# microsoft/AI2BMD

Hardware: NVIDIA H100
Metric: MD steps/sec (higher is better)
Workload: dtype f32

## Files before the change

ai2bmd_b200/csrc/engine.cu:

```cuda
#include <cuda_runtime.h>
#include <cxxabi.h>

#include <algorithm>
#include <cmath>
#include <cstdarg>
#include <cstdio>
#include <cstdlib>
#include <cstring>
#include <mutex>
#include <string>
#include <vector>

#include "../../include/visnet_b200.h"
#include "k_edge.cuh"
#include "k_caph.cuh"
#include "k_comm.cuh"
#include "k_edge_tc.cuh"
#include "k_graph_embed.cuh"
#include <nvtx3/nvToolsExt.h>
#include "k_head.cuh"
#include "k_md.cuh"
#include "k_nonbonded.cuh"
#include "k_node.cuh"
#include "k_node2.cuh"
// ... 383 lines not shown
    const int blocks = std::max(1, std::min(tiles, h->sm_count * occ));
    Lc.launch(edge_fwd_kernel<TE, NW>, dim3(blocks), dim3(NW * 32), edge_fwd_smem_bytes<TE>(), a);
    Lc.check();
}
template <int TE, int NW>
void launch_edge_bwd(Launcher& Lc, int l, int occ) {
    vb_handle* h = Lc.h;
    EdgeArgs a{l, h->mw, h->ws};
    const int tiles = (h->ws.Ecap + TE - 1) / TE;
    const int blocks = std::max(1, std::min(tiles, h->sm_count * occ));
    Lc.launch(edge_bwd_kernel<TE, NW>, dim3(blocks), dim3(NW * 32), edge_bwd_smem_bytes<TE>(), a);
    Lc.check();
}

template <int NB>
void launch_node_fwd2(Launcher& Lc, int k) {
    vb_handle* h = Lc.h;
    NodeArgs a{k, h->mw, h->ws, h->timeline ? h->d_tl + (size_t)2 * L * TC_TL_SLOTS + (size_t)k * N2_TL_SLOTS : nullptr, h->krot};
    Lc.launch(node_fwd2_kernel<NB>, dim3((h->ws.N + NB - 1) / NB), dim3(N2Cfg<NB>::THREADS), sizeof(NodeFwd2Smem<NB>), a);
    Lc.check();
}
template <int NB>
void launch_node_bwd2(Launcher& Lc, int k) {
    vb_handle* h = Lc.h;
    NodeArgs a{k, h->mw, h->ws, h->timeline ? h->d_tl + (size_t)2 * L * TC_TL_SLOTS + (size_t)(L + 1 + k) * N2_TL_SLOTS : nullptr, h->krot};
    Lc.launch(node_bwd2_kernel<NB>, dim3((h->ws.N + NB - 1) / NB), dim3(N2Cfg<NB>::THREADS), sizeof(NodeBwd2Smem<NB>), a);
    Lc.check();
}
int node_nb(const vb_handle* h) {
    if (h->node_nb > 0) return h->node_nb;
    for (int nb = 1; nb <= 4; nb++)
        if ((h->ws.N + nb - 1) / nb <= h->sm_count) return nb;
    return 8;
}
void node_fwd(Launcher& Lc, int k) {
    if (Lc.h->npw == 2) launch_node_fwd2<16>(Lc, k);
    else switch (node_nb(Lc.h)) {
        case 1: launch_node_fwd2<1>(Lc, k); break;
        case 2: launch_node_fwd2<2>(Lc, k); break;
        case 3: launch_node_fwd2<3>(Lc, k); break;
        case 4: launch_node_fwd2<4>(Lc, k); break;
        default: launch_node_fwd2<8>(Lc, k);
    }
}
void node_bwd(Launcher& Lc, int k) {
    switch (node_nb(Lc.h)) {
        case 1: launch_node_bwd2<1>(Lc, k); break;
        case 2: launch_node_bwd2<2>(Lc, k); break;
        case 3: launch_node_bwd2<3>(Lc, k); break;
        case 4: launch_node_bwd2<4>(Lc, k); break;
        default: launch_node_bwd2<8>(Lc, k);
    }
}
void head(Launcher& Lc) {
    vb_handle* h = Lc.h;
    if (h->ws.N <= 4096) {
        Lc.launch(head2_kernel, dim3(h->ws.N), dim3(128), 0, h->mw, h->ws);
        Lc.check();
        return;
    }
    h->npw == 2 ? launch_head<2>(Lc) : launch_head<1>(Lc);
}
void launch_edge_fwd_tc(Launcher& Lc, int l) {
    vb_handle* h = Lc.h;
    EdgeTcArgs a{};
    a.layer = l; a.mw = h->mw; a.ws = h->ws;
    const LayerW& lw = h->mw.layer[l];
    const size_t chunk = 4 * 8192;
    int n = 0;
    a.jobs[n++] = TcJob{lw.tcW1, 0};
    a.jobs[n++] = TcJob{lw.tcW1 + chunk, 0};
    if (l < L - 1) a.jobs[n++] = TcJob{lw.tcW1 + 2 * chunk, 0};
    a.jobs[n++] = TcJob{lw.tcWs, 0};
    a.jobs[n++] = TcJob{lw.tcWs + chunk, 0};
    a.njobs = n;
    a.tl = h->timeline ? h->d_tl + (size_t)l * TC_TL_SLOTS : nullptr;
    a.tile_rows = h->tile_rows;
    const int rows = h->tc_rows;
    const int tiles = (h->ws.Ecap + h->tile_rows - 1) / h->tile_rows;
    const int blocks = std::max(1, std::min(tiles, h->sm_count));
    if (rows == 32) Lc.launch(edge_fwd_tc_kernel<32>, dim3(blocks), dim3(TC2_THREADS), TC_SMEM_BYTES, a);
    else if (rows == 64) Lc.launch(edge_fwd_tc_kernel<64>, dim3(blocks), dim3(TC2_THREADS), TC_SMEM_BYTES, a);
    else if (rows == 96) Lc.launch(edge_fwd_tc_kernel<96>, dim3(blocks), dim3(TC2_THREADS), TC_SMEM_BYTES, a);
    else Lc.launch(edge_fwd_tc_kernel<128>, dim3(blocks), dim3(TC2_THREADS), TC_SMEM_BYTES, a);
    Lc.check();
}

void edge_fwd(Launcher& Lc, int l) {
    if (Lc.h->edge_tc & 1) { launch_edge_fwd_tc(Lc, l); return; }
    if (Lc.h->te_fwd == 64) launch_edge_fwd<64, 8>(Lc, l, 2);
    else launch_edge_fwd<32, 8>(Lc, l, 4);
}
void launch_edge_bwd_tc(Launcher& Lc, int l) {
    vb_handle* h = Lc.h;
    EdgeTcArgs a{};
    a.layer = l; a.mw = h->mw; a.ws = h->ws;
    const LayerW& lw = h->mw.layer[l];
    const size_t chunk = 4 * 8192;
    const bool upd = l < L - 1;
    int n = 0;
    a.jobs[n++] = TcJob{lw.tcWsN, 0};
    a.jobs[n++] = TcJob{lw.tcWsN + chunk, 1};
    a.jobs[n++] = TcJob{lw.tcW1N + chunk, 0};
    a.jobs[n++] = TcJob{lw.tcW1N, 1};
    if (upd) a.jobs[n++] = TcJob{lw.tcW1N + 2 * chunk, 1};
    a.njobs = n;
    a.tl = h->timeline ? h->d_tl + (size_t)(L + l) * TC_TL_SLOTS : nullptr;
    a.tile_rows = h->tile_rows;
    const int rows = h->tc_rows;
    const int tiles = (h->ws.Ecap + h->tile_rows - 1) / h->tile_rows;
// ... 134 lines not shown
            node_fwd_tc(Lc, l);
            snprintf(name, sizeof(name), "edge_fwd%d", l);
            if (Lc.next(name)) edge_fwd(Lc, l);
        }
        node_fwd_tc(Lc, L);
        if (Lc.next("head")) head(Lc);
        for (int l = L - 1; l >= 0; l--) {
            node_bwd_tc(Lc, l + 1);
            snprintf(name, sizeof(name), "edge_bwd%d", l);
            if (Lc.next(name)) edge_bwd(Lc, l);
        }
        node_bwd_tc(Lc, 0);
    } else {
        for (int l = 0; l < L; l++) {
            snprintf(name, sizeof(name), "node_fwd%d", l);
            if (Lc.next(name)) node_fwd(Lc, l);
            snprintf(name, sizeof(name), "edge_fwd%d", l);
            if (Lc.next(name)) edge_fwd(Lc, l);
        }
        if (Lc.next("node_fwd6")) node_fwd(Lc, L);
        if (Lc.next("head")) head(Lc);
        for (int l = L - 1; l >= 0; l--) {
            snprintf(name, sizeof(name), "node_bwd%d", l + 1);
            if (Lc.next(name)) node_bwd(Lc, l + 1);
            snprintf(name, sizeof(name), "edge_bwd%d", l);
            if (Lc.next(name)) edge_bwd(Lc, l);
        }
        if (Lc.next("node_bwd0")) node_bwd(Lc, 0);
    }
    if (Lc.next("embed_edge_bwd")) {
        const int bb = std::max(1, std::min((ws.Ecap + EEB_WARPS - 1) / EEB_WARPS, h->sm_count * 4));
        Lc.launch(embed_edge_bwd_kernel, dim3(bb), dim3(EEB_WARPS * 32), 0, h->mw, ws);
        Lc.check();
    }
    if (Lc.next("embed_node_bwd")) {
        Lc.launch(embed_node_bwd_kernel, dim3(batch_bwd ? std::min(N, 5 * h->sm_count) : N), dim3(ENB_WARPS * 32), 0, h->mw, ws, io.forces);
        Lc.check();
    }
    if (Lc.next("finalize")) enqueue_finalize(Lc, io);
}

template <typename K>
cudaError_t opt_in_smem(K kernel, size_t bytes) {
    return cudaFuncSetAttribute(kernel, cudaFuncAttributeMaxDynamicSharedMemorySize, (int)bytes);
}

int configure_kernels(vb_handle* h) {
    CUDA_TRY(h, opt_in_smem(edge_fwd_kernel<32, 8>, edge_fwd_smem_bytes<32>()));
    CUDA_TRY(h, opt_in_smem(edge_fwd_kernel<64, 8>, edge_fwd_smem_bytes<64>()));
    CUDA_TRY(h, opt_in_smem(edge_bwd_kernel<32, 8>, edge_bwd_smem_bytes<32>()));
    CUDA_TRY(h, opt_in_smem(edge_bwd_kernel<64, 8>, edge_bwd_smem_bytes<64>()));
    CUDA_TRY(h, opt_in_smem(head_kernel<1>, HeadSmem<1>::BYTES));
    CUDA_TRY(h, opt_in_smem(head_kernel<2>, HeadSmem<2>::BYTES));
    CUDA_TRY(h, opt_in_smem(edge_fwd_tc_kernel<32>, TC_SMEM_BYTES));
    CUDA_TRY(h, opt_in_smem(edge_fwd_tc_kernel<64>, TC_SMEM_BYTES));
    CUDA_TRY(h, opt_in_smem(edge_fwd_tc_kernel<96>, TC_SMEM_BYTES));
    CUDA_TRY(h, opt_in_smem(edge_fwd_tc_kernel<128>, TC_SMEM_BYTES));
    CUDA_TRY(h, opt_in_smem(edge_bwd_tc_kernel<32>, TC_SMEM_BYTES));
    CUDA_TRY(h, opt_in_smem(edge_bwd_tc_kernel<64>, TC_SMEM_BYTES));
    CUDA_TRY(h, opt_in_smem(edge_bwd_tc_kernel<96>, TC_SMEM_BYTES));
    CUDA_TRY(h, opt_in_smem(edge_bwd_tc_kernel<128>, TC_SMEM_BYTES));
    CUDA_TRY(h, opt_in_smem(node_tc_kernel<NT_OPROJ>, TC_SMEM_BYTES));
    CUDA_TRY(h, opt_in_smem(node_tc_kernel<NT_PROJ>, TC_SMEM_BYTES));
    CUDA_TRY(h, opt_in_smem(node_tc_kernel<NT_BWDA>, TC_SMEM_BYTES));
    CUDA_TRY(h, opt_in_smem(node_tc_kernel<NT_BWDB>, TC_SMEM_BYTES));

    CUDA_TRY(h, opt_in_smem(node_fwd2_kernel<1>, sizeof(NodeFwd2Smem<1>)));
    CUDA_TRY(h, opt_in_smem(node_bwd2_kernel<1>, sizeof(NodeBwd2Smem<1>)));
    CUDA_TRY(h, opt_in_smem(node_fwd2_kernel<2>, sizeof(NodeFwd2Smem<2>)));
    CUDA_TRY(h, opt_in_smem(node_bwd2_kernel<2>, sizeof(NodeBwd2Smem<2>)));
    CUDA_TRY(h, opt_in_smem(node_fwd2_kernel<3>, sizeof(NodeFwd2Smem<3>)));
    CUDA_TRY(h, opt_in_smem(node_bwd2_kernel<3>, sizeof(NodeBwd2Smem<3>)));
    CUDA_TRY(h, opt_in_smem(node_fwd2_kernel<4>, sizeof(NodeFwd2Smem<4>)));
    CUDA_TRY(h, opt_in_smem(node_bwd2_kernel<4>, sizeof(NodeBwd2Smem<4>)));
    CUDA_TRY(h, opt_in_smem(node_fwd2_kernel<8>, sizeof(NodeFwd2Smem<8>)));
    CUDA_TRY(h, opt_in_smem(node_fwd2_kernel<16>, sizeof(NodeFwd2Smem<16>)));
    CUDA_TRY(h, opt_in_smem(node_bwd2_kernel<8>, sizeof(NodeBwd2Smem<8>)));
    return VB_OK;
}

int clean_accumulators(vb_handle* h, cudaStream_t st) {
    const Workspace& ws = h->ws;
    const size_t N = ws.N;
    CUDA_TRY(h, cudaMemsetAsync(ws.XA, 0, N * D * 4, st));
    CUDA_TRY(h, cudaMemsetAsync(ws.VA, 0, N * 3 * D * 4, st));
    CUDA_TRY(h, cudaMemsetAsync(ws.GQKV, 0, N * 3 * D * 4, st));
    CUDA_TRY(h, cudaMemsetAsync(ws.GVNMSG, 0, N * 3 * D * 4, st));
    CUDA_TRY(h, cudaMemsetAsync(ws.GTU, 0, N * 6 * D * 4, st));
    CUDA_TRY(h, cudaMemsetAsync(ws.GX, 0, N * D * 4, st));
    CUDA_TRY(h, cudaMemsetAsync(ws.GXA, 0, 3 * N * D * 4, st));
    h->accum_dirty = false;
    return VB_OK;
}

enum { K_EVAL = 0, K_HOST = 1, K_MD_EVAL = 2, K_MD_STEP = 3 };

template <typename F>
int run_cached(vb_handle* h, cudaStream_t st, int kind, const StepIO& io, F&& enqueue) {
    if (h->accum_dirty) { if (int rc = clean_accumulators(h, st)) return rc; }
    if (!h->use_graph) return enqueue(st);
    for (auto& g : h->graphs)
        if (g.kind == kind && g.io == io) { CUDA_TRY(h, cudaGraphLaunch(g.exec, st)); return VB_OK; }
    cudaGraphExec_t exec = nullptr;
    for (int attempt = 0; attempt < 2 && !exec; attempt++) {
        cudaGraph_t graph = nullptr;
        CUDA_TRY(h, cudaStreamBeginCapture(h->own_stream, cudaStreamCaptureModeThreadLocal));
// ... 1206 lines not shown
```

ai2bmd_b200/csrc/k_head.cuh:

```cuda
#pragma once
#include "k_node.cuh"

namespace vb {

template <int NPW>
struct HeadSmem {
    static constexpr int L128 = D + LDS_PAD;
    static constexpr int L256 = 2 * D + LDS_PAD;
    static constexpr int L64 = 64 + LDS_PAD;
    static constexpr int OFF_VS = 0;
    static constexpr int OFF_CAT = OFF_VS + 3 * NPW * L128;
    static constexpr int OFF_HS = OFF_CAT + NPW * L256;
    static constexpr int OFF_YS = OFF_HS + NPW * L128;
    static constexpr int OFF_VP = OFF_YS + NPW * L128;
    static constexpr int OFF_CB = OFF_VP + 3 * NPW * L64;
    static constexpr int OFF_GPB = OFF_CB + NPW * L128;
    static constexpr int OFF_GPRE = OFF_GPB + NPW * L64;
    static constexpr int PER_WARP = OFF_GPRE + NPW * L128;
    static constexpr size_t BYTES = (size_t)NODE_WARPS * PER_WARP * sizeof(float);
};

template <int NPW>
__global__ void __launch_bounds__(NODE_WARPS * 32) head_kernel(ModelW mw, Workspace ws) {
    pdl_entry();
    using S = HeadSmem<NPW>;
    constexpr int L128 = S::L128, L256 = S::L256, L64 = S::L64;
    extern __shared__ __align__(16) float dyn_smem[];
    const int lane = threadIdx.x & 31, warp = threadIdx.x >> 5;
    float* sm = dyn_smem + (size_t)warp * S::PER_WARP;
    float* Vs = sm + S::OFF_VS;
    float* cat = sm + S::OFF_CAT;
    float* hs = sm + S::OFF_HS;
    float* ys = sm + S::OFF_YS;
    float* Vp = sm + S::OFF_VP;
    float* cb = sm + S::OFF_CB;
    float* gpb = sm + S::OFF_GPB;
    float* gpre = sm + S::OFF_GPRE;
    const int n0 = (blockIdx.x * NODE_WARPS + warp) * NPW;
    if (n0 >= ws.N) return;
    const int col = lane * 4, c2 = lane * 2;
    const float stdv = __ldg(mw.scalars);

    float4 x6[NPW], v6[NPW][3];
#pragma unroll
    for (int nd = 0; nd < NPW; nd++) {
        const int node = n0 + nd;
        const bool ok = node < ws.N;
        x6[nd] = ok ? ld4(ws.X[L] + (size_t)node * D + col) : f4s(0.f);
#pragma unroll
        for (int s = 0; s < 3; s++) v6[nd][s] = ok ? ld4(ws.V[L] + ((size_t)node * 3 + s) * D + col) : f4s(0.f);
        st4(cat + nd * L256 + col, ln_forward(x6[nd], mw.on_w, mw.on_b, lane));
        float4 vn[3];
        vecln_forward(v6[nd], vn, mw.von_w, lane);
// ... 112 lines not shown
            float gg = 0.f;
#pragma unroll
            for (int s = 0; s < 3; s++) {
                gg += gVp[nd * 3 + s][q] * p2[nd * 3 + s][q];
                Vp[(nd * 3 + s) * L64 + c2 + q] = gVp[nd * 3 + s][q] * gate[nd][q];
            }
            hs[nd * L128 + 64 + c2 + q] = gg;
            hs[nd * L128 + c2 + q] = cb[nd * L128 + c2 + q] * dsilu_(ys[nd * L128 + c2 + q]);
        }
    }
    __syncwarp();
    {
        float gh[NPW][4];
        acc_zero<NPW>(gh);
        warp_gemm<NPW, D, L128>(gh, hs, mw.h0_U2N, D, lane);
#pragma unroll
        for (int nd = 0; nd < NPW; nd++) st4(gpre + nd * L128 + col, arr4(gh[nd]) * dsilu4(arr4(pre[nd])));
    }
    __syncwarp();
    float gX[NPW][4], gn1[NPW][4];
    acc_zero<NPW>(gX);
    acc_zero<NPW>(gn1);
    warp_gemm<NPW, D, L128>(gX, gpre, mw.h0_U0N, 2 * D, lane);
    warp_gemm<NPW, D, L128>(gn1, gpre, mw.h0_U0N + D, 2 * D, lane);
#pragma unroll
    for (int nd = 0; nd < NPW; nd++) {
        const float4 g = arr4(gn1[nd]);
        const float4 sc = f4(n1[nd].x > 0.f ? g.x / n1[nd].x : 0.f, n1[nd].y > 0.f ? g.y / n1[nd].y : 0.f,
                             n1[nd].z > 0.f ? g.z / n1[nd].z : 0.f, n1[nd].w > 0.f ? g.w / n1[nd].w : 0.f);
#pragma unroll
        for (int s = 0; s < 3; s++) st4(Vs + (nd * 3 + s) * L128 + col, sc * arr4(p1[nd * 3 + s]));
    }
    __syncwarp();
    float gV[3 * NPW][4];
    acc_zero<3 * NPW>(gV);
    warp_gemm<3 * NPW, D, L128>(gV, Vs, mw.h0_W1N, D, lane);
    warp_gemm<3 * NPW, 64, L64>(gV, Vp, mw.h0_W2N, D, lane);
#pragma unroll
    for (int nd = 0; nd < NPW; nd++) {
        const int node = n0 + nd;
        if (node >= ws.N) continue;
        float4 gout[3], gv[3];
#pragma unroll
        for (int s = 0; s < 3; s++) gout[s] = arr4(gV[nd * 3 + s]);
        vecln_backward(v6[nd], gout, gv, mw.von_w, lane);
#pragma unroll
        for (int s = 0; s < 3; s++) st4(ws.GVEC + ((size_t)node * 3 + s) * D + col, gv[s]);
        st4(ws.GX + (size_t)node * D + col, ln_backward(x6[nd], arr4(gX[nd]), mw.on_w, lane));
    }
}

}

namespace vb {

struct Head2Smem {
    static constexpr int L128 = D + LDS_PAD, L256 = 2 * D + LDS_PAD, L64 = 64 + LDS_PAD;
    float Vs[3][L128];
    float cat[L256];
    float hs[L128];
    float ys[L128];
    float Vp[3][L64];
    float cb[L128];
    float gpb[L64];
    float gpre[L128];
    float red[4][3][D];
};

template <int R, int K, int LDA>
__device__ __forceinline__ void ksplit_gemm(float (&acc)[R][4], const float* As, const float* __restrict__ W, int ldw,
                                            int lane, int warp, float (&red)[4][3][D]) {
    float part[R][4];
    acc_zero<R>(part);
    warp_gemm<R, K / 4, LDA, 4>(part, As + warp * (K / 4), W + (size_t)warp * (K / 4) * ldw, ldw, lane);
#pragma unroll
    for (int r = 0; r < R; r++) st4(&red[warp][r][lane * 4], arr4(part[r]));
    __syncthreads();
#pragma unroll
    for (int r = 0; r < R; r++) {
        const float4 s = (ld4(&red[0][r][lane * 4]) + ld4(&red[1][r][lane * 4])) + (ld4(&red[2][r][lane * 4]) + ld4(&red[3][r][lane * 4]));
        acc[r][0] += s.x; acc[r][1] += s.y; acc[r][2] += s.z; acc[r][3] += s.w;
    }
    __syncthreads();
}
template <int R, int K, int LDA>
__device__ __forceinline__ void ksplit_gemm2(float (&acc)[R][2], const float* As, const float* __restrict__ W, int ldw,
                                             int lane, int warp, float (&red)[4][3][D]) {
    float part[R][2];
#pragma unroll
    for (int r = 0; r < R; r++) part[r][0] = part[r][1] = 0.f;
    warp_gemm2<R, K / 4, LDA>(part, As + warp * (K / 4), W + (size_t)warp * (K / 4) * ldw, ldw, lane);
#pragma unroll
    for (int r = 0; r < R; r++) { red[warp][r][lane * 2] = part[r][0]; red[warp][r][lane * 2 + 1] = part[r][1]; }
    __syncthreads();
#pragma unroll
    for (int r = 0; r < R; r++) {
        acc[r][0] += (red[0][r][lane * 2] + red[1][r][lane * 2]) + (red[2][r][lane * 2] + red[3][r][lane * 2]);
        acc[r][1] += (red[0][r][lane * 2 + 1] + red[1][r][lane * 2 + 1]) + (red[2][r][lane * 2 + 1] + red[3][r][lane * 2 + 1]);
    }
    __syncthreads();
}

__global__ void __launch_bounds__(128) head2_kernel(ModelW mw, Workspace ws) {
    pdl_entry();
    constexpr int L128 = Head2Smem::L128, L256 = Head2Smem::L256, L64 = Head2Smem::L64;
    __shared__ __align__(16) Head2Smem sm;
    const int lane = threadIdx.x & 31, warp = threadIdx.x >> 5;
    const int node = blockIdx.x;
    if (node >= ws.N) return;
    const int col = lane * 4, c2 = lane * 2;
    const bool w0 = (warp == 0);
    const float stdv = __ldg(mw.scalars);

    float4 x6 = ld4(ws.X[L] + (size_t)node * D + col), v6[3];
#pragma unroll
    for (int s = 0; s < 3; s++) v6[s] = ld4(ws.V[L] + ((size_t)node * 3 + s) * D + col);
    {
        const float4 xn = ln_forward(x6, mw.on_w, mw.on_b, lane);
        float4 vn[3];
        vecln_forward(v6, vn, mw.von_w, lane);
        if (w0) {
            st4(&sm.cat[col], xn);
#pragma unroll
            for (int s = 0; s < 3; s++) st4(&sm.Vs[s][col], vn[s]);
        }
    }
    __syncthreads();
    float p1[3][4], p2[3][2];
    acc_zero<3>(p1);
    ksplit_gemm<3, D, L128>(p1, &sm.Vs[0][0], mw.h0_W1T, D, lane, warp, sm.red);
#pragma unroll
    for (int r = 0; r < 3; r++) p2[r][0] = p2[r][1] = 0.f;
    ksplit_gemm2<3, D, L128>(p2, &sm.Vs[0][0], mw.h0_W2T, 64, lane, warp, sm.red);
    float4 n1;
    {
        const float4 a = arr4(p1[0]), b = arr4(p1[1]), c = arr4(p1[2]);
        const float4 q = a * a + b * b + c * c;
        n1 = f4(sqrtf(q.x), sqrtf(q.y), sqrtf(q.z), sqrtf(q.w));
        if (w0) st4(&sm.cat[D + col], n1);
    }
    __syncthreads();
    float pre[1][4];
    acc_set_bias<1>(pre, mw.h0_b0, lane);
    ksplit_gemm<1, 2 * D, L256>(pre, &sm.cat[0], mw.h0_U0T, D, lane, warp, sm.red);
    if (w0) st4(&sm.hs[col], silu4(arr4(pre[0])));
    __syncthreads();
    {
        float y[1][4];
        acc_set_bias<1>(y, mw.h0_b2, lane);
        ksplit_gemm<1, D, L128>(y, &sm.hs[0], mw.h0_U2T, D, lane, warp, sm.red);
        if (w0) st4(&sm.ys[col], arr4(y[0]));
    }
    __syncthreads();
    float gate[2];
    gate[0] = sm.ys[64 + c2];
    gate[1] = sm.ys[64 + c2 + 1];
    if (w0) {
        sm.cb[c2] = silu_(sm.ys[c2]);
        sm.cb[c2 + 1] = silu_(sm.ys[c2 + 1]);
#pragma unroll
        for (int s = 0; s < 3; s++) {
            sm.Vp[s][c2] = gate[0] * p2[s][0];
            sm.Vp[s][c2 + 1] = gate[1] * p2[s][1];
        }
    }
    __syncthreads();
    float p1b[3][2];
#pragma unroll
    for (int r = 0; r < 3; r++) p1b[r][0] = p1b[r][1] = 0.f;
    ksplit_gemm2<3, 64, L64>(p1b, &sm.Vp[0][0], mw.h1_W1T, 64, lane, warp, sm.red);
    float n1b[2];
#pragma unroll
    for (int q = 0; q < 2; q++) {
        n1b[q] = sqrtf(p1b[0][q] * p1b[0][q] + p1b[1][q] * p1b[1][q] + p1b[2][q] * p1b[2][q]);
        if (w0) sm.cb[64 + c2 + q] = n1b[q];
    }
    __syncthreads();
    float preb[1][2];
    {
        const float2 bb = __ldg(reinterpret_cast<const float2*>(mw.h1_b0 + c2));
        preb[0][0] = bb.x; preb[0][1] = bb.y;
    }
    ksplit_gemm2<1, D, L128>(preb, &sm.cb[0], mw.h1_U0T, 64, lane, warp, sm.red);
    const float2 u2 = __ldg(reinterpret_cast<const float2*>(mw.h1_u2 + c2));
    {
        const float e = warp_sum(silu_(preb[0][0]) * u2.x + silu_(preb[0][1]) * u2.y) + __ldg(mw.h1_b2);
        if (threadIdx.x == 0) ws.eatom[node] = e * stdv + __ldg(mw.atomref + ws.z[node]);
    }
    if (w0) {
        sm.gpb[c2] = stdv * u2.x * dsilu_(preb[0][0]);
        sm.gpb[c2 + 1] = stdv * u2.y * dsilu_(preb[0][1]);
    }
    __syncthreads();
    {
        float gcb[1][4];
        acc_zero<1>(gcb);
        ksplit_gemm<1, 64, L64>(gcb, &sm.gpb[0], mw.h1_U0N, D, lane, warp, sm.red);
        if (w0) st4(&sm.cb[col], arr4(gcb[0]));
    }
    __syncthreads();
    if (w0) {
#pragma unroll
        for (int q = 0; q < 2; q++) {
            const float gn = sm.cb[64 + c2 + q];
            const float sc = n1b[q] > 0.f ? gn / n1b[q] : 0.f;
#pragma unroll
            for (int s = 0; s < 3; s++) sm.Vp[s][c2 + q] = sc * p1b[s][q];
        }
    }
    __syncthreads();
    float gVp[3][2];
#pragma unroll
    for (int r = 0; r < 3; r++) gVp[r][0] = gVp[r][1] = 0.f;
    ksplit_gemm2<3, 64, L64>(gVp, &sm.Vp[0][0], mw.h1_W1N, 64, lane, warp, sm.red);
    if (w0) {
#pragma unroll
        for (int q = 0; q < 2; q++) {
            float gg = 0.f;
#pragma unroll
            for (int s = 0; s < 3; s++) {
                gg += gVp[s][q] * p2[s][q];
                sm.Vp[s][c2 + q] = gVp[s][q] * gate[q];
            }
            sm.hs[64 + c2 + q] = gg;
            sm.hs[c2 + q] = sm.cb[c2 + q] * dsilu_(sm.ys[c2 + q]);
        }
    }
    __syncthreads();
    {
        float gh[1][4];
        acc_zero<1>(gh);
        ksplit_gemm<1, D, L128>(gh, &sm.hs[0], mw.h0_U2N, D, lane, warp, sm.red);
        if (w0) st4(&sm.gpre[col], arr4(gh[0]) * dsilu4(arr4(pre[0])));
    }
    __syncthreads();
    float gX[1][4], gn1[1][4];
    acc_zero<1>(gX);
    acc_zero<1>(gn1);
    ksplit_gemm<1, D, L128>(gX, &sm.gpre[0], mw.h0_U0N, 2 * D, lane, warp, sm.red);
    ksplit_gemm<1, D, L128>(gn1, &sm.gpre[0], mw.h0_U0N + D, 2 * D, lane, warp, sm.red);
    if (w0) {
        const float4 g = arr4(gn1[0]);
        const float4 sc = f4(n1.x > 0.f ? g.x / n1.x : 0.f, n1.y > 0.f ? g.y / n1.y : 0.f, n1.z > 0.f ? g.z / n1.z : 0.f,
                             n1.w > 0.f ? g.w / n1.w : 0.f);
#pragma unroll
        for (int s = 0; s < 3; s++) st4(&sm.Vs[s][col], sc * arr4(p1[s]));
    }
    __syncthreads();
    float gV[3][4];
    acc_zero<3>(gV);
    ksplit_gemm<3, D, L128>(gV, &sm.Vs[0][0], mw.h0_W1N, D, lane, warp, sm.red);
    ksplit_gemm<3, 64, L64>(gV, &sm.Vp[0][0], mw.h0_W2N, D, lane, warp, sm.red);
    if (w0) {
        float4 gout[3], gv[3];
#pragma unroll
        for (int s = 0; s < 3; s++) gout[s] = arr4(gV[s]);
        vecln_backward(v6, gout, gv, mw.von_w, lane);
#pragma unroll
        for (int s = 0; s < 3; s++) st4(ws.GVEC + ((size_t)node * 3 + s) * D + col, gv[s]);
        st4(ws.GX + (size_t)node * D + col, ln_backward(x6, arr4(gX[0]), mw.on_w, lane));
    }
}

}
```

Baseline: 1154.

## Batch multiple nodes per head2 block with k-split 16-warp GEMMs and weight prefetch

Measured after the change: 1163 (median of 6 runs). No clear change (+0.7%).

```diff
diff --git a/ai2bmd_b200/csrc/engine.cu b/ai2bmd_b200/csrc/engine.cu
--- a/ai2bmd_b200/csrc/engine.cu
+++ b/ai2bmd_b200/csrc/engine.cu
@@ -459,10 +459,17 @@
         default: launch_node_bwd2<8>(Lc, k);
     }
 }
+int head_nb(const vb_handle* h) {
+    for (int nb = 1; nb < HEAD2_MAX_NB; nb++)
+        if ((h->ws.N + nb - 1) / nb <= h->sm_count) return nb;
+    return HEAD2_MAX_NB;
+}
 void head(Launcher& Lc) {
     vb_handle* h = Lc.h;
     if (h->ws.N <= 4096) {
-        Lc.launch(head2_kernel, dim3(h->ws.N), dim3(128), 0, h->mw, h->ws);
+        const int nb = head_nb(h);
+        Lc.launch(head2_kernel, dim3((h->ws.N + nb - 1) / nb), dim3(HEAD2_WARPS * 32), sizeof(Head2Smem), h->mw, h->ws,
+                  nb, h->krot);
         Lc.check();
         return;
     }
@@ -703,6 +710,7 @@
     CUDA_TRY(h, opt_in_smem(edge_bwd_kernel<64, 8>, edge_bwd_smem_bytes<64>()));
     CUDA_TRY(h, opt_in_smem(head_kernel<1>, HeadSmem<1>::BYTES));
     CUDA_TRY(h, opt_in_smem(head_kernel<2>, HeadSmem<2>::BYTES));
+    CUDA_TRY(h, opt_in_smem(head2_kernel, sizeof(Head2Smem)));
     CUDA_TRY(h, opt_in_smem(edge_fwd_tc_kernel<32>, TC_SMEM_BYTES));
     CUDA_TRY(h, opt_in_smem(edge_fwd_tc_kernel<64>, TC_SMEM_BYTES));
     CUDA_TRY(h, opt_in_smem(edge_fwd_tc_kernel<96>, TC_SMEM_BYTES));
diff --git a/ai2bmd_b200/csrc/k_head.cuh b/ai2bmd_b200/csrc/k_head.cuh
--- a/ai2bmd_b200/csrc/k_head.cuh
+++ b/ai2bmd_b200/csrc/k_head.cuh
@@ -1,4 +1,5 @@
 #pragma once
+#include <type_traits>
 #include "k_node.cuh"
 
 namespace vb {
@@ -217,214 +218,376 @@
 
 }
 
+
 namespace vb {
 
+constexpr int HEAD2_WARPS = 16, HEAD2_MAX_NB = 8;
+
 struct Head2Smem {
+    static constexpr int NB = HEAD2_MAX_NB, RV = 3 * NB;
     static constexpr int L128 = D + LDS_PAD, L256 = 2 * D + LDS_PAD, L64 = 64 + LDS_PAD;
-    float Vs[3][L128];
-    float cat[L256];
-    float hs[L128];
-    float ys[L128];
-    float Vp[3][L64];
-    float cb[L128];
-    float gpb[L64];
-    float gpre[L128];
-    float red[4][3][D];
+    static constexpr int RED = 4 * RV * 192;
+    float red[RED];
+    float Vs[RV][L128];
+    float cat[NB][L256];
+    float p1[RV][D];
+    float p2[RV][64];
+    float pre[NB][D];
+    float hs[NB][L128];
+    float ys[NB][D];
+    float Vp[RV][L64];
+    float p1b[RV][64];
+    float cb[NB][L128];
+    float gpb[NB][L64];
+    float gpre[NB][L128];
+    float gx[NB][D];
 };
 
-template <int R, int K, int LDA>
-__device__ __forceinline__ void ksplit_gemm(float (&acc)[R][4], const float* As, const float* __restrict__ W, int ldw,
-                                            int lane, int warp, float (&red)[4][3][D]) {
-    float part[R][4];
-    acc_zero<R>(part);
-    warp_gemm<R, K / 4, LDA, 4>(part, As + warp * (K / 4), W + (size_t)warp * (K / 4) * ldw, ldw, lane);
-#pragma unroll
-    for (int r = 0; r < R; r++) st4(&red[warp][r][lane * 4], arr4(part[r]));
-    __syncthreads();
-#pragma unroll
-    for (int r = 0; r < R; r++) {
-        const float4 s = (ld4(&red[0][r][lane * 4]) + ld4(&red[1][r][lane * 4])) + (ld4(&red[2][r][lane * 4]) + ld4(&red[3][r][lane * 4]));
-        acc[r][0] += s.x; acc[r][1] += s.y; acc[r][2] += s.z; acc[r][3] += s.w;
-    }
-    __syncthreads();
-}
-template <int R, int K, int LDA>
-__device__ __forceinline__ void ksplit_gemm2(float (&acc)[R][2], const float* As, const float* __restrict__ W, int ldw,
-                                             int lane, int warp, float (&red)[4][3][D]) {
-    float part[R][2];
-#pragma unroll
-    for (int r = 0; r < R; r++) part[r][0] = part[r][1] = 0.f;
-    warp_gemm2<R, K / 4, LDA>(part, As + warp * (K / 4), W + (size_t)warp * (K / 4) * ldw, ldw, lane);
-#pragma unroll
-    for (int r = 0; r < R; r++) { red[warp][r][lane * 2] = part[r][0]; red[warp][r][lane * 2 + 1] = part[r][1]; }
-    __syncthreads();
-#pragma unroll
-    for (int r = 0; r < R; r++) {
-        acc[r][0] += (red[0][r][lane * 2] + red[1][r][lane * 2]) + (red[2][r][lane * 2] + red[3][r][lane * 2]);
-        acc[r][1] += (red[0][r][lane * 2 + 1] + red[1][r][lane * 2 + 1]) + (red[2][r][lane * 2 + 1] + red[3][r][lane * 2 + 1]);
-    }
-    __syncthreads();
-}
-
-__global__ void __launch_bounds__(128) head2_kernel(ModelW mw, Workspace ws) {
+__device__ __forceinline__ void head_fma(float (&c)[4], float a, float4 w) {
+    c[0] = fmaf(a, w.x, c[0]); c[1] = fmaf(a, w.y, c[1]); c[2] = fmaf(a, w.z, c[2]); c[3] = fmaf(a, w.w, c[3]);
+}
+__device__ __forceinline__ void head_fma(float (&c)[2], float a, float2 w) {
+    c[0] = fmaf(a, w.x, c[0]); c[1] = fmaf(a, w.y, c[1]);
+}
+__device__ __forceinline__ void head_park(float* p, const float (&c)[4]) { st4(p, arr4(c)); }
+__device__ __forceinline__ void head_park(float* p, const float (&c)[2]) { *reinterpret_cast<float2*>(p) = make_float2(c[0], c[1]); }
+
+template <int KU, int CW, int NPRE>
+struct HeadUnit {
+    static_assert((KU & (KU - 1)) == 0 && KU % (4 * NPRE) == 0, "KU: power of two and a multiple of the ring");
+    static_assert(CW == 4 || CW == 2, "4 or 2 columns per lane");
+    using VT = typename std::conditional<CW == 4, float4, float2>::type;
+    VT w[NPRE][4];
+    const float* Wp;
+    int ldw, krot;
+    __device__ __forceinline__ int kk(int k) const { return (k + krot) & (KU - 1); }
+    __device__ __forceinline__ void load(VT (&g)[4], int k) const {
+#pragma unroll
+        for (int j = 0; j < 4; j++) g[j] = __ldg(reinterpret_cast<const VT*>(Wp + (size_t)(k + j) * ldw));
+    }
+    __device__ __forceinline__ void prefetch(const float* __restrict__ W, int ldw_, int lane, int krot_) {
+        Wp = W + lane * CW; ldw = ldw_; krot = krot_;
+#pragma unroll
+        for (int g = 0; g < NPRE; g++) load(w[g], kk(4 * g));
+    }
+    __device__ __forceinline__ void restart() {
+#pragma unroll
+        for (int g = 0; g < NPRE; g++) load(w[g], kk(4 * g));
+    }
+    template <int R, int LDA>
+    __device__ __forceinline__ void run(float (&acc)[R][CW], const float* __restrict__ As) {
+#pragma unroll 1
+        for (int k = 0; k < KU; k += 4 * NPRE) {
+#pragma unroll
+            for (int g = 0; g < NPRE; g++) {
+                const int k0 = kk(k + 4 * g);
+#pragma unroll
+                for (int r = 0; r < R; r++) {
+                    const float4 a = ld4(As + r * LDA + k0);
+                    head_fma(acc[r], a.x, w[g][0]); head_fma(acc[r], a.y, w[g][1]);
+                    head_fma(acc[r], a.z, w[g][2]); head_fma(acc[r], a.w, w[g][3]);
+                }
+                if (k + 4 * (g + NPRE) < KU) load(w[g], kk(k + 4 * (g + NPRE)));
+            }
+        }
+    }
+};
+
+template <int R, int CW>
+__device__ __forceinline__ void head_zero(float (&acc)[R][CW]) {
+#pragma unroll
+    for (int r = 0; r < R; r++)
+#pragma unroll
+        for (int j = 0; j < CW; j++) acc[r][j] = 0.f;
+}
+template <int RT, int R, int CW, int WD>
+__device__ __forceinline__ void head_park_rows(float* red, int sl, int r0, int c0, int lane, const float (&acc)[R][CW]) {
+#pragma unroll
+    for (int r = 0; r < R; r++) head_park(red + ((size_t)sl * RT + r0 + r) * WD + c0 + lane * CW, acc[r]);
+}
+template <int R, int CW, int WD>
+__device__ __forceinline__ void head_park_rows(float* red, int sl, int c0, int lane, const float (&acc)[R][CW]) {
+    head_park_rows<R, R, CW, WD>(red, sl, 0, c0, lane, acc);
+}
+template <int RV, int LDA, int WD, int KU, int NPRE>
+__device__ __forceinline__ void head_vec_unit(HeadUnit<KU, 2, NPRE>& u, const float* As, float* red, int sl, int c0, int lane) {
+    if constexpr (RV <= 12) {
+        float acc[RV][2];
+        head_zero(acc);
+        u.template run<RV, LDA>(acc, As);
+        head_park_rows<RV, RV, 2, WD>(red, sl, 0, c0, lane, acc);
+    } else {
+        constexpr int R0 = (RV + 1) / 2, R1 = RV - R0;
+        {
+            float acc[R0][2];
+            head_zero(acc);
+            u.template run<R0, LDA>(acc, As);
+            head_park_rows<RV, R0, 2, WD>(red, sl, 0, c0, lane, acc);
+        }
+        u.restart();
+        float acc[R1][2];
+        head_zero(acc);
+        u.template run<R1, LDA>(acc, As + R0 * LDA);
+        head_park_rows<RV, R1, 2, WD>(red, sl, R0, c0, lane, acc);
+    }
+}
+template <int S>
+__device__ __forceinline__ float head_sum(const float* p, int stride) {
+    float v = p[0];
+#pragma unroll
+    for (int s = 1; s < S; s++) v += p[s * stride];
+    return v;
+}
+
+template <int NB>
+__device__ __forceinline__ void head2_body(const ModelW& mw, const Workspace& ws, Head2Smem& sm, int krot) {
+    constexpr int RV = 3 * NB, NT = HEAD2_WARPS * 32;
+    constexpr int L128 = Head2Smem::L128, L256 = Head2Smem::L256, L64 = Head2Smem::L64;
+    const int lane = threadIdx.x & 31, warp = threadIdx.x >> 5, col = lane * 4;
+    const int n0 = (int)blockIdx.x * NB, nn = min(NB, ws.N - n0);
+    if (nn <= 0) return;
+    const float stdv = __ldg(mw.scalars);
+    float* const red = sm.red;
+    constexpr int PV = 2, PS = 2;
+
+    HeadUnit<32, 2, PV> u_p;
+    if (warp < 12) {
+        const int ch = warp % 3, sl = warp / 3;
+        if (ch < 2) u_p.prefetch(mw.h0_W1T + (size_t)sl * 32 * D + ch * 64, D, lane, krot);
+        else        u_p.prefetch(mw.h0_W2T + (size_t)sl * 32 * 64, 64, lane, krot);
+    }
+    if (warp < NB) {
+        const int nd = warp;
+        if (nd < nn) {
+            const int node = n0 + nd;
+            const float4 x6 = ld4(ws.X[L] + (size_t)node * D + col);
+            float4 v6[3], vn[3];
+#pragma unroll
+            for (int s = 0; s < 3; s++) v6[s] = ld4(ws.V[L] + ((size_t)node * 3 + s) * D + col);
+            st4(&sm.cat[nd][col], ln_forward(x6, mw.on_w, mw.on_b, lane));
+            vecln_forward(v6, vn, mw.von_w, lane);
+#pragma unroll
+            for (int s = 0; s < 3; s++) st4(&sm.Vs[nd * 3 + s][col], vn[s]);
+        } else {
+            st4(&sm.cat[nd][col], f4s(0.f));
+#pragma unroll
+            for (int s = 0; s < 3; s++) st4(&sm.Vs[nd * 3 + s][col], f4s(0.f));
+        }
+    }
+    __syncthreads();
+    if (warp < 12) {
+        const int ch = warp % 3, sl = warp / 3;
+        head_vec_unit<RV, L128, 192>(u_p, &sm.Vs[0][sl * 32], red, sl, ch * 64, lane);
+    }
+    HeadUnit<16, 4, PS> u_u0;
+    u_u0.prefetch(mw.h0_U0T + (size_t)warp * 16 * D, D, lane, krot);
+    __syncthreads();
+    for (int idx = threadIdx.x; idx < NB * 192; idx += NT) {
+        const int nd = idx / 192, c = idx % 192;
+        float v[3];
+#pragma unroll
+        for (int s = 0; s < 3; s++) v[s] = head_sum<4>(red + (nd * 3 + s) * 192 + c, RV * 192);
+        if (c < D) {
+#pragma unroll
+            for (int s = 0; s < 3; s++) sm.p1[nd * 3 + s][c] = v[s];
+            sm.cat[nd][D + c] = sqrtf(v[0] * v[0] + v[1] * v[1] + v[2] * v[2]);
+        } else {
+#pragma unroll
+            for (int s = 0; s < 3; s++) sm.p2[nd * 3 + s][c - D] = v[s];
+        }
+    }
+    __syncthreads();
+    {
+        float acc[NB][4];
+        head_zero(acc);
+        u_u0.template run<NB, L256>(acc, &sm.cat[0][warp * 16]);
+        head_park_rows<NB, 4, D>(red, warp, 0, lane, acc);
+    }
+    HeadUnit<8, 4, 2> u_u2;
+    u_u2.prefetch(mw.h0_U2T + (size_t)warp * 8 * D, D, lane, krot);
+    __syncthreads();
+    for (int idx = threadIdx.x; idx < NB * D; idx += NT) {
+        const int nd = idx / D, c = idx % D;
+        const float pre = __ldg(mw.h0_b0 + c) + head_sum<16>(red + nd * D + c, NB * D);
+        sm.pre[nd][c] = pre;
+        sm.hs[nd][c] = silu_(pre);
+    }
+    __syncthreads();
+    {
+        float acc[NB][4];
+        head_zero(acc);
+        u_u2.template run<NB, L128>(acc, &sm.hs[0][warp * 8]);
+        head_park_rows<NB, 4, D>(red, warp, 0, lane, acc);
+    }
+    HeadUnit<8, 2, 2> u_w1b;
+    if (warp < 8) u_w1b.prefetch(mw.h1_W1T + (size_t)warp * 8 * 64, 64, lane, krot);
+    __syncthreads();
+    for (int idx = threadIdx.x; idx < NB * D; idx += NT) {
+        const int nd = idx / D, c = idx % D;
+        const float y = __ldg(mw.h0_b2 + c) + head_sum<16>(red + nd * D + c, NB * D);
+        sm.ys[nd][c] = y;
+        if (c < 64) {
+            sm.cb[nd][c] = silu_(y);
+        } else {
+#pragma unroll
+            for (int s = 0; s < 3; s++) sm.Vp[nd * 3 + s][c - 64] = y * sm.p2[nd * 3 + s][c - 64];
+        }
+    }
+    __syncthreads();
+    if (warp < 8) head_vec_unit<RV, L64, 64>(u_w1b, &sm.Vp[0][warp * 8], red, warp, 0, lane);
+    HeadUnit<8, 2, 2> u_u0b;
+    u_u0b.prefetch(mw.h1_U0T + (size_t)warp * 8 * 64, 64, lane, krot);
+    __syncthreads();
+    for (int idx = threadIdx.x; idx < NB * 64; idx += NT) {
+        const int nd = idx / 64, c = idx % 64;
+        float v[3];
+#pragma unroll
+        for (int s = 0; s < 3; s++) {
+            v[s] = head_sum<8>(red + (nd * 3 + s) * 64 + c, RV * 64);
+            sm.p1b[nd * 3 + s][c] = v[s];
+        }
+        sm.cb[nd][64 + c] = sqrtf(v[0] * v[0] + v[1] * v[1] + v[2] * v[2]);
+    }
+    __syncthreads();
+    {
+        float acc[NB][2];
+        head_zero(acc);
+        u_u0b.template run<NB, L128>(acc, &sm.cb[0][warp * 8]);
+        head_park_rows<NB, 2, 64>(red, warp, 0, lane, acc);
+    }
+    HeadUnit<4, 4, 1> u_u0bn;
+    u_u0bn.prefetch(mw.h1_U0N + (size_t)warp * 4 * D, D, lane, krot);
+    __syncthreads();
+    if (warp < NB) {
+        const int nd = warp, c2 = lane * 2;
+        const float2 bb = __ldg(reinterpret_cast<const float2*>(mw.h1_b0 + c2));
+        const float preb0 = bb.x + head_sum<16>(red + nd * 64 + c2, NB * 64);
+        const float preb1 = bb.y + head_sum<16>(red + nd * 64 + c2 + 1, NB * 64);
+        const float2 u2 = __ldg(reinterpret_cast<const float2*>(mw.h1_u2 + c2));
+        const float e = warp_sum(silu_(preb0) * u2.x + silu_(preb1) * u2.y) + __ldg(mw.h1_b2);
+        if (lane == 0 && nd < nn) ws.eatom[n0 + nd] = e * stdv + __ldg(mw.atomref + ws.z[n0 + nd]);
+        sm.gpb[nd][c2] = stdv * u2.x * dsilu_(preb0);
+        sm.gpb[nd][c2 + 1] = stdv * u2.y * dsilu_(preb1);
+    }
+    __syncthreads();
+    {
+        float acc[NB][4];
+        head_zero(acc);
+        u_u0bn.template run<NB, L64>(acc, &sm.gpb[0][warp * 4]);
+        head_park_rows<NB, 4, D>(red, warp, 0, lane, acc);
+    }
+    HeadUnit<8, 2, 2> u_w1bn;
+    if (warp < 8) u_w1bn.prefetch(mw.h1_W1N + (size_t)warp * 8 * 64, 64, lane, krot);
+    __syncthreads();
+    for (int idx = threadIdx.x; idx < NB * D; idx += NT) {
+        const int nd = idx / D, c = idx % D;
+        const float g = head_sum<16>(red + nd * D + c, NB * D);
+        if (c < 64) {
+            sm.cb[nd][c] = g;
+        } else {
+            const float n1b = sm.cb[nd][c];
+            const float sc = n1b > 0.f ? g / n1b : 0.f;
+#pragma unroll
+            for (int s = 0; s < 3; s++) sm.Vp[nd * 3 + s][c - 64] = sc * sm.p1b[nd * 3 + s][c - 64];
+        }
+    }
+    __syncthreads();
+    if (warp < 8) head_vec_unit<RV, L64, 64>(u_w1bn, &sm.Vp[0][warp * 8], red, warp, 0, lane);
+    HeadUnit<8, 4, 2> u_u2n;
+    u_u2n.prefetch(mw.h0_U2N + (size_t)warp * 8 * D, D, lane, krot);
+    __syncthreads();
+    for (int idx = threadIdx.x; idx < NB * 64; idx += NT) {
+        const int nd = idx / 64, c = idx % 64;
+        const float gate = sm.ys[nd][64 + c];
+        float gg = 0.f;
+#pragma unroll
+        for (int s = 0; s < 3; s++) {
+            const float gvp = head_sum<8>(red + (nd * 3 + s) * 64 + c, RV * 64);
+            gg += gvp * sm.p2[nd * 3 + s][c];
+            sm.Vp[nd * 3 + s][c] = gvp * gate;
+        }
+        sm.hs[nd][64 + c] = gg;
+        sm.hs[nd][c] = sm.cb[nd][c] * dsilu_(sm.ys[nd][c]);
+    }
+    __syncthreads();
+    {
+        float acc[NB][4];
+        head_zero(acc);
+        u_u2n.template run<NB, L128>(acc, &sm.hs[0][warp * 8]);
+        head_park_rows<NB, 4, D>(red, warp, 0, lane, acc);
+    }
+    HeadUnit<16, 4, PS> u_u0n;
+    u_u0n.prefetch(mw.h0_U0N + (size_t)(warp >> 1) * 16 * 2 * D + (warp & 1) * D, 2 * D, lane, krot);
+    __syncthreads();
+    for (int idx = threadIdx.x; idx < NB * D; idx += NT) {
+        const int nd = idx / D, c = idx % D;
+        sm.gpre[nd][c] = head_sum<16>(red + nd * D + c, NB * D) * dsilu_(sm.pre[nd][c]);
+    }
+    __syncthreads();
+    {
+        float acc[NB][4];
+        head_zero(acc);
+        u_u0n.template run<NB, L128>(acc, &sm.gpre[0][(warp >> 1) * 16]);
+        head_park_rows<NB, 4, 2 * D>(red, warp >> 1, (warp & 1) * D, lane, acc);
+    }
+    HeadUnit<32, 2, PV> u_wn;
+    if (warp < 12) {
+        const int ch = warp & 1, sl = warp >> 1;
+        if (sl < 4) u_wn.prefetch(mw.h0_W1N + (size_t)sl * 32 * D + ch * 64, D, lane, krot);
+        else        u_wn.prefetch(mw.h0_W2N + (size_t)(sl - 4) * 32 * D + ch * 64, D, lane, krot);
+    }
+    __syncthreads();
+    for (int idx = threadIdx.x; idx < NB * 2 * D; idx += NT) {
+        const int nd = idx / (2 * D), c = idx % (2 * D);
+        const float g = head_sum<8>(red + nd * 2 * D + c, NB * 2 * D);
+        if (c < D) {
+            sm.gx[nd][c] = g;
+        } else {
+            const float n1 = sm.cat[nd][c];
+            const float sc = n1 > 0.f ? g / n1 : 0.f;
+#pragma unroll
+            for (int s = 0; s < 3; s++) sm.Vs[nd * 3 + s][c - D] = sc * sm.p1[nd * 3 + s][c - D];
+        }
+    }
+    __syncthreads();
+    if (warp < 12) {
+        const int ch = warp & 1, sl = warp >> 1;
+        if (sl < 4) head_vec_unit<RV, L128, D>(u_wn, &sm.Vs[0][sl * 32], red, sl, ch * 64, lane);
+        else        head_vec_unit<RV, L64, D>(u_wn, &sm.Vp[0][(sl - 4) * 32], red, sl, ch * 64, lane);
+    }
+    __syncthreads();
+    if (warp < nn) {
+        const int nd = warp, node = n0 + nd;
+        const float4 x6 = ld4(ws.X[L] + (size_t)node * D + col);
+        float4 v6[3], gout[3], gv[3];
+#pragma unroll
+        for (int s = 0; s < 3; s++) {
+            v6[s] = ld4(ws.V[L] + ((size_t)node * 3 + s) * D + col);
+            const float* p = red + (nd * 3 + s) * D + col;
+            gout[s] = f4(head_sum<6>(p, RV * D), head_sum<6>(p + 1, RV * D), head_sum<6>(p + 2, RV * D), head_sum<6>(p + 3, RV * D));
+        }
+        vecln_backward(v6, gout, gv, mw.von_w, lane);
+#pragma unroll
+        for (int s = 0; s < 3; s++) st4(ws.GVEC + ((size_t)node * 3 + s) * D + col, gv[s]);
+        st4(ws.GX + (size_t)node * D + col, ln_backward(x6, ld4(&sm.gx[nd][col]), mw.on_w, lane));
+    }
+}
+
+__global__ void __launch_bounds__(HEAD2_WARPS * 32, 1) head2_kernel(ModelW mw, Workspace ws, int nb, int krot) {
     pdl_entry();
-    constexpr int L128 = Head2Smem::L128, L256 = Head2Smem::L256, L64 = Head2Smem::L64;
-    __shared__ __align__(16) Head2Smem sm;
-    const int lane = threadIdx.x & 31, warp = threadIdx.x >> 5;
-    const int node = blockIdx.x;
-    if (node >= ws.N) return;
-    const int col = lane * 4, c2 = lane * 2;
-    const bool w0 = (warp == 0);
-    const float stdv = __ldg(mw.scalars);
-
-    float4 x6 = ld4(ws.X[L] + (size_t)node * D + col), v6[3];
-#pragma unroll
-    for (int s = 0; s < 3; s++) v6[s] = ld4(ws.V[L] + ((size_t)node * 3 + s) * D + col);
-    {
-        const float4 xn = ln_forward(x6, mw.on_w, mw.on_b, lane);
-        float4 vn[3];
-        vecln_forward(v6, vn, mw.von_w, lane);
-        if (w0) {
-            st4(&sm.cat[col], xn);
-#pragma unroll
-            for (int s = 0; s < 3; s++) st4(&sm.Vs[s][col], vn[s]);
-        }
-    }
-    __syncthreads();
-    float p1[3][4], p2[3][2];
-    acc_zero<3>(p1);
-    ksplit_gemm<3, D, L128>(p1, &sm.Vs[0][0], mw.h0_W1T, D, lane, warp, sm.red);
-#pragma unroll
-    for (int r = 0; r < 3; r++) p2[r][0] = p2[r][1] = 0.f;
-    ksplit_gemm2<3, D, L128>(p2, &sm.Vs[0][0], mw.h0_W2T, 64, lane, warp, sm.red);
-    float4 n1;
-    {
-        const float4 a = arr4(p1[0]), b = arr4(p1[1]), c = arr4(p1[2]);
-        const float4 q = a * a + b * b + c * c;
-        n1 = f4(sqrtf(q.x), sqrtf(q.y), sqrtf(q.z), sqrtf(q.w));
-        if (w0) st4(&sm.cat[D + col], n1);
-    }
-    __syncthreads();
-    float pre[1][4];
-    acc_set_bias<1>(pre, mw.h0_b0, lane);
-    ksplit_gemm<1, 2 * D, L256>(pre, &sm.cat[0], mw.h0_U0T, D, lane, warp, sm.red);
-    if (w0) st4(&sm.hs[col], silu4(arr4(pre[0])));
-    __syncthreads();
-    {
-        float y[1][4];
-        acc_set_bias<1>(y, mw.h0_b2, lane);
-        ksplit_gemm<1, D, L128>(y, &sm.hs[0], mw.h0_U2T, D, lane, warp, sm.red);
-        if (w0) st4(&sm.ys[col], arr4(y[0]));
-    }
-    __syncthreads();
-    float gate[2];
-    gate[0] = sm.ys[64 + c2];
-    gate[1] = sm.ys[64 + c2 + 1];
-    if (w0) {
-        sm.cb[c2] = silu_(sm.ys[c2]);
-        sm.cb[c2 + 1] = silu_(sm.ys[c2 + 1]);
-#pragma unroll
-        for (int s = 0; s < 3; s++) {
-            sm.Vp[s][c2] = gate[0] * p2[s][0];
-            sm.Vp[s][c2 + 1] = gate[1] * p2[s][1];
-        }
-    }
-    __syncthreads();
-    float p1b[3][2];
-#pragma unroll
-    for (int r = 0; r < 3; r++) p1b[r][0] = p1b[r][1] = 0.f;
-    ksplit_gemm2<3, 64, L64>(p1b, &sm.Vp[0][0], mw.h1_W1T, 64, lane, warp, sm.red);
-    float n1b[2];
-#pragma unroll
-    for (int q = 0; q < 2; q++) {
-        n1b[q] = sqrtf(p1b[0][q] * p1b[0][q] + p1b[1][q] * p1b[1][q] + p1b[2][q] * p1b[2][q]);
-        if (w0) sm.cb[64 + c2 + q] = n1b[q];
-    }
-    __syncthreads();
-    float preb[1][2];
-    {
-        const float2 bb = __ldg(reinterpret_cast<const float2*>(mw.h1_b0 + c2));
-        preb[0][0] = bb.x; preb[0][1] = bb.y;
-    }
-    ksplit_gemm2<1, D, L128>(preb, &sm.cb[0], mw.h1_U0T, 64, lane, warp, sm.red);
-    const float2 u2 = __ldg(reinterpret_cast<const float2*>(mw.h1_u2 + c2));
-    {
-        const float e = warp_sum(silu_(preb[0][0]) * u2.x + silu_(preb[0][1]) * u2.y) + __ldg(mw.h1_b2);
-        if (threadIdx.x == 0) ws.eatom[node] = e * stdv + __ldg(mw.atomref + ws.z[node]);
-    }
-    if (w0) {
-        sm.gpb[c2] = stdv * u2.x * dsilu_(preb[0][0]);
-        sm.gpb[c2 + 1] = stdv * u2.y * dsilu_(preb[0][1]);
-    }
-    __syncthreads();
-    {
-        float gcb[1][4];
-        acc_zero<1>(gcb);
-        ksplit_gemm<1, 64, L64>(gcb, &sm.gpb[0], mw.h1_U0N, D, lane, warp, sm.red);
-        if (w0) st4(&sm.cb[col], arr4(gcb[0]));
-    }
-    __syncthreads();
-    if (w0) {
-#pragma unroll
-        for (int q = 0; q < 2; q++) {
-            const float gn = sm.cb[64 + c2 + q];
-            const float sc = n1b[q] > 0.f ? gn / n1b[q] : 0.f;
-#pragma unroll
-            for (int s = 0; s < 3; s++) sm.Vp[s][c2 + q] = sc * p1b[s][q];
-        }
-    }
-    __syncthreads();
-    float gVp[3][2];
-#pragma unroll
-    for (int r = 0; r < 3; r++) gVp[r][0] = gVp[r][1] = 0.f;
-    ksplit_gemm2<3, 64, L64>(gVp, &sm.Vp[0][0], mw.h1_W1N, 64, lane, warp, sm.red);
-    if (w0) {
-#pragma unroll
-        for (int q = 0; q < 2; q++) {
-            float gg = 0.f;
-#pragma unroll
-            for (int s = 0; s < 3; s++) {
-                gg += gVp[s][q] * p2[s][q];
-                sm.Vp[s][c2 + q] = gVp[s][q] * gate[q];
-            }
-            sm.hs[64 + c2 + q] = gg;
-            sm.hs[c2 + q] = sm.cb[c2 + q] * dsilu_(sm.ys[c2 + q]);
-        }
-    }
-    __syncthreads();
-    {
-        float gh[1][4];
-        acc_zero<1>(gh);
-        ksplit_gemm<1, D, L128>(gh, &sm.hs[0], mw.h0_U2N, D, lane, warp, sm.red);
-        if (w0) st4(&sm.gpre[col], arr4(gh[0]) * dsilu4(arr4(pre[0])));
-    }
-    __syncthreads();
-    float gX[1][4], gn1[1][4];
-    acc_zero<1>(gX);
-    acc_zero<1>(gn1);
-    ksplit_gemm<1, D, L128>(gX, &sm.gpre[0], mw.h0_U0N, 2 * D, lane, warp, sm.red);
-    ksplit_gemm<1, D, L128>(gn1, &sm.gpre[0], mw.h0_U0N + D, 2 * D, lane, warp, sm.red);
-    if (w0) {
-        const float4 g = arr4(gn1[0]);
-        const float4 sc = f4(n1.x > 0.f ? g.x / n1.x : 0.f, n1.y > 0.f ? g.y / n1.y : 0.f, n1.z > 0.f ? g.z / n1.z : 0.f,
-                             n1.w > 0.f ? g.w / n1.w : 0.f);
-#pragma unroll
-        for (int s = 0; s < 3; s++) st4(&sm.Vs[s][col], sc * arr4(p1[s]));
-    }
-    __syncthreads();
-    float gV[3][4];
-    acc_zero<3>(gV);
-    ksplit_gemm<3, D, L128>(gV, &sm.Vs[0][0], mw.h0_W1N, D, lane, warp, sm.red);
-    ksplit_gemm<3, 64, L64>(gV, &sm.Vp[0][0], mw.h0_W2N, D, lane, warp, sm.red);
-    if (w0) {
-        float4 gout[3], gv[3];
-#pragma unroll
-        for (int s = 0; s < 3; s++) gout[s] = arr4(gV[s]);
-        vecln_backward(v6, gout, gv, mw.von_w, lane);
-#pragma unroll
-        for (int s = 0; s < 3; s++) st4(ws.GVEC + ((size_t)node * 3 + s) * D + col, gv[s]);
-        st4(ws.GX + (size_t)node * D + col, ln_backward(x6, arr4(gX[0]), mw.on_w, lane));
-    }
-}
-
-}
+    extern __shared__ __align__(16) float dyn_smem[];
+    Head2Smem& sm = *reinterpret_cast<Head2Smem*>(dyn_smem);
+    const int kr = krot ? (int)blockIdx.x * 4 : 0;
+    switch (nb) {
+        case 1: head2_body<1>(mw, ws, sm, kr); break;
+        case 2: head2_body<2>(mw, ws, sm, kr); break;
+        case 3: head2_body<3>(mw, ws, sm, kr); break;
+        case 4: head2_body<4>(mw, ws, sm, kr); break;
+        case 5: head2_body<5>(mw, ws, sm, kr); break;
+        case 6: head2_body<6>(mw, ws, sm, kr); break;
+        case 7: head2_body<7>(mw, ws, sm, kr); break;
+        default: head2_body<8>(mw, ws, sm, kr);
+    }
+}
+
+}
```
